# sebrahimi1988/dss-ml-at-scale

Hardware: AMD Instinct MI355X
Metric: samples/sec (higher is better)
Workload: dtype bf16; 1 GPU; model=resnet18, global_batch=212, parallelism=dp1+hipgraph

## Files before the change

mi355x_scale/models/resnet.py:

```python
from __future__ import annotations

from typing import List, Optional, Type, Union

import torch
import torch.nn as nn

from ..ops.conv3x3 import Conv3x3
from ..ops.fused_bn import FusedBNReLU2d
from ..ops.maxpool import MaxPool3x3s2
from ..ops.stemconv import StemConv2d


def _conv3x3(cin: int, cout: int, stride: int = 1) -> nn.Conv2d:
    if stride == 1 and cin == cout:
        return Conv3x3(cin, cout)
    return nn.Conv2d(cin, cout, 3, stride=stride, padding=1, bias=False)


def _conv1x1(cin: int, cout: int, stride: int = 1) -> nn.Conv2d:
    return nn.Conv2d(cin, cout, 1, stride=stride, bias=False)


class BasicBlock(nn.Module):
    expansion = 1
# ... 48 lines not shown
        self.layer3 = self._make_layer(block, 256, layers[2], stride=2)
        self.layer4 = self._make_layer(block, 512, layers[3], stride=2)
        self.avgpool = nn.AdaptiveAvgPool2d(1)
        self.fc = nn.Linear(512 * block.expansion, num_classes)

        for m in self.modules():
            if isinstance(m, nn.Conv2d):
                nn.init.kaiming_normal_(m.weight, mode="fan_out",
                                        nonlinearity="relu")
            elif isinstance(m, nn.BatchNorm2d):
                nn.init.ones_(m.weight)
                nn.init.zeros_(m.bias)
        if zero_init_residual:
            for m in self.modules():
                if isinstance(m, Bottleneck):
                    nn.init.zeros_(m.bn3.weight)
                elif isinstance(m, BasicBlock):
                    nn.init.zeros_(m.bn2.weight)

    def _make_layer(self, block, planes: int, blocks: int,
                    stride: int = 1) -> nn.Sequential:
        downsample = None
        if stride != 1 or self.inplanes != planes * block.expansion:
            downsample = nn.Sequential(
                _conv1x1(self.inplanes, planes * block.expansion, stride),
                FusedBNReLU2d(planes * block.expansion, relu=False),
            )
        layers = [block(self.inplanes, planes, stride, downsample)]
        self.inplanes = planes * block.expansion
        layers += [block(self.inplanes, planes) for _ in range(1, blocks)]
        return nn.Sequential(*layers)

    def forward(self, x: torch.Tensor) -> torch.Tensor:
        x = self.bn1.forward_pooled(self.conv1(x))
        x = self.layer4(self.layer3(self.layer2(self.layer1(x))))
        x = self.avgpool(x).flatten(1)
        return self.fc(x)


def resnet18(num_classes: int = 1000) -> ResNet:
    return ResNet(BasicBlock, [2, 2, 2, 2], num_classes)


def resnet34(num_classes: int = 1000) -> ResNet:
    return ResNet(BasicBlock, [3, 4, 6, 3], num_classes)


def resnet50(num_classes: int = 1000) -> ResNet:
    return ResNet(Bottleneck, [3, 4, 6, 3], num_classes)


MODELS = {"resnet18": resnet18, "resnet34": resnet34, "resnet50": resnet50}


def build_model(name: str, num_classes: int = 1000) -> ResNet:
    try:
        return MODELS[name](num_classes)
    except KeyError:
        raise ValueError(f"unknown model {name!r}; have {sorted(MODELS)}")
```

mi355x_scale/ops/csrc/bindings.cpp:

```cpp

#include <torch/extension.h>
#include <ATen/hip/HIPContext.h>
#include <hip/hip_runtime.h>

extern "C" void launch_normalize_u8_to_bf16(
    const uint8_t* in, void* out, const float* scale_dev,
    const float* shift_dev, long long n, hipStream_t stream);

void normalize_u8_to_bf16(torch::Tensor in, torch::Tensor out,
                          torch::Tensor scale, torch::Tensor shift) {
  TORCH_CHECK(in.is_cuda() && out.is_cuda(), "tensors must be on GPU");
  TORCH_CHECK(in.scalar_type() == torch::kUInt8, "input must be uint8");
  TORCH_CHECK(out.scalar_type() == torch::kBFloat16, "output must be bf16");
  TORCH_CHECK(in.is_contiguous(), "input must be contiguous (NHWC)");
  TORCH_CHECK(in.numel() == out.numel(), "element count mismatch");
  TORCH_CHECK(scale.is_cuda() && shift.is_cuda() && scale.numel() == 3 &&
                  shift.numel() == 3,
              "scale/shift must be 3-element device float tensors");
  TORCH_CHECK(scale.scalar_type() == torch::kFloat32 &&
              shift.scalar_type() == torch::kFloat32,
              "scale/shift must be float32");
  auto stream = at::cuda::getCurrentHIPStream();
  launch_normalize_u8_to_bf16(
      in.data_ptr<uint8_t>(), out.data_ptr(),
      scale.data_ptr<float>(), shift.data_ptr<float>(),
      (long long)in.numel(), stream.stream());
}

extern "C" void launch_groupfit_eval(
    const float* yT, const float* xc0, const float* xc1, const float* xc2,
    const float* pj0, const float* pj1, const float* pj2, const int* orders,
    float* mse, unsigned char* statusv,
    const float* b0, const float* b1, const float* b2,
    const float* w0, const float* w1, const float* w2,
    int T, long long G, int S, int C,
    int KX, hipStream_t stream);

extern "C" void launch_diff_center(const float* yT, float* wc, float* wm,
                                   int T, long long G, int S, int d,
                                   hipStream_t stream);

extern "C" void launch_exog_project_mfma(const float* P, const float* wc,
                                         float* beta, int n, long long G,
                                         int KX, hipStream_t stream);

extern "C" void launch_groupfit_final(
    const float* yT, const float* xc0, const float* xc1, const float* xc2,
    const float* pj0, const float* pj1, const float* pj2,
    const int* best_order, float* fitted, float* params,
    unsigned char* statusv,
    const float* b0, const float* b1, const float* b2,
    const float* w0, const float* w1, const float* w2,
    int T, long long G, int KX, hipStream_t stream);

extern "C" void launch_stem_conv_fwd(const void* x, const void* w, void* out,
                                     void* wp_scratch,
                                     int Nb, int H, int W, int HO, int WO,
                                     hipStream_t stream, int phase_mask);
extern "C" void launch_stem_conv_wrw(const void* x, const void* dy,
                                     float* dw_f32, void* dw_bf16,
                                     int Nb, int H, int W, int HO, int WO,
                                     hipStream_t stream, int phase_mask);
extern "C" void launch_conv3x3_wrw(const void* x, const void* dy,
                                   float* part, void* dw_bf16,
                                   int Nb, int H, int W, int C,
                                   int chunks, hipStream_t stream,
                                   int phase_mask);
extern "C" int conv3x3_wrw_chunks(int Nb, int H, int C, int chunks_req);

static void _check_f32(const torch::Tensor& t, const char* name) {
  TORCH_CHECK(t.is_cuda() && t.scalar_type() == torch::kFloat32 &&
                  t.is_contiguous(),
              name, " must be contiguous f32 on GPU");
}

void groupfit_eval(torch::Tensor yT, torch::Tensor xc0, torch::Tensor xc1,
                   torch::Tensor xc2, torch::Tensor pj0, torch::Tensor pj1,
                   torch::Tensor pj2, torch::Tensor orders,
                   torch::Tensor mse, torch::Tensor status, int64_t S,
                   torch::Tensor b0, torch::Tensor b1, torch::Tensor b2,
                   torch::Tensor w0, torch::Tensor w1, torch::Tensor w2) {
  _check_f32(yT, "yT"); _check_f32(xc0, "xc0"); _check_f32(xc1, "xc1");
  _check_f32(xc2, "xc2"); _check_f32(pj0, "pj0"); _check_f32(pj1, "pj1");
  _check_f32(pj2, "pj2"); _check_f32(mse, "mse");
  TORCH_CHECK(orders.scalar_type() == torch::kInt32 && orders.is_cuda());
  TORCH_CHECK(status.scalar_type() == torch::kUInt8 && status.is_cuda());
  int T = yT.size(0);
  long long G = yT.size(1);
  int C = orders.size(0);
  TORCH_CHECK(S > 8 && S <= T, "need 8 < S <= T");
  TORCH_CHECK(mse.size(0) == C && mse.size(1) == G);
// ... 490 lines not shown
                   at::cuda::getCurrentHIPStream().stream());
}

extern "C" void launch_adam_step_mixed(float* master, const void* gb,
                                       const float* gf, float* m, float* v,
                                       void* pb, int* step, float lr,
                                       float beta1, float beta2, float eps,
                                       float weight_decay, long long nb,
                                       long long n, hipStream_t stream);

void adam_step_mixed(torch::Tensor master, torch::Tensor gb,
                     torch::Tensor gf, torch::Tensor m, torch::Tensor v,
                     torch::Tensor pb, torch::Tensor step, double lr,
                     double beta1, double beta2, double eps,
                     double weight_decay) {
  _check_f32(master, "master"); _check_f32(m, "m"); _check_f32(v, "v");
  TORCH_CHECK(gb.scalar_type() == torch::kBFloat16 &&
              pb.scalar_type() == torch::kBFloat16, "gb/pb must be bf16");
  TORCH_CHECK(step.is_cuda() && step.scalar_type() == torch::kInt32 &&
              step.numel() == 1, "step must be int32[1] on device");
  long long n = master.numel();
  long long nb = gb.numel();
  TORCH_CHECK(pb.numel() == nb && gf.numel() == n - nb &&
              m.numel() == n && v.numel() == n, "buffer length mismatch");
  const float* gf_p = gf.numel() ? gf.data_ptr<float>() : nullptr;
  launch_adam_step_mixed(master.data_ptr<float>(), gb.data_ptr(), gf_p,
                         m.data_ptr<float>(), v.data_ptr<float>(),
                         pb.data_ptr(), step.data_ptr<int>(), (float)lr,
                         (float)beta1, (float)beta2, (float)eps,
                         (float)weight_decay, nb, n,
                         at::cuda::getCurrentHIPStream().stream());
}

void stem_conv_fwd(torch::Tensor x, torch::Tensor w, torch::Tensor out,
                   torch::Tensor wp_scratch, int64_t phase_mask = 7) {
  TORCH_CHECK(x.is_cuda() && x.scalar_type() == torch::kBFloat16);
  TORCH_CHECK(w.is_cuda() && w.scalar_type() == torch::kBFloat16);
  TORCH_CHECK(out.is_cuda() && out.scalar_type() == torch::kBFloat16);
  int Nb = x.size(0), H = x.size(1), W = x.size(2);
  TORCH_CHECK(x.size(3) == 3 && out.size(3) == 64, "stem is 3->64");
  int HO = out.size(1), WO = out.size(2);
  TORCH_CHECK(WO <= 128, "stem kernel handles output rows up to 128 px");
  TORCH_CHECK(w.numel() == 64 * 7 * 7 * 3);
  TORCH_CHECK(wp_scratch.scalar_type() == torch::kBFloat16 &&
              wp_scratch.numel() == 64 * 160);
  launch_stem_conv_fwd(x.data_ptr(), w.data_ptr(), out.data_ptr(),
                       wp_scratch.data_ptr(),
                       Nb, H, W, HO, WO,
                       at::cuda::getCurrentHIPStream().stream(),
                       (int)phase_mask);
}

void stem_conv_wrw(torch::Tensor x, torch::Tensor dy, torch::Tensor dw_f32,
                   torch::Tensor dw, int64_t phase_mask = 7) {
  TORCH_CHECK(x.is_cuda() && x.scalar_type() == torch::kBFloat16);
  TORCH_CHECK(dy.is_cuda() && dy.scalar_type() == torch::kBFloat16);
  TORCH_CHECK(dw_f32.scalar_type() == torch::kFloat32 &&
              dw_f32.numel() == 64 * 160);
  TORCH_CHECK(dw.scalar_type() == torch::kBFloat16 &&
              dw.numel() == 64 * 7 * 7 * 3);
  int Nb = x.size(0), H = x.size(1), W = x.size(2);
  int HO = dy.size(1), WO = dy.size(2);
  launch_stem_conv_wrw(x.data_ptr(), dy.data_ptr(),
                       dw_f32.data_ptr<float>(), dw.data_ptr(),
                       Nb, H, W, HO, WO,
                       at::cuda::getCurrentHIPStream().stream(),
                       (int)phase_mask);
}

void conv3x3_wrw(torch::Tensor x, torch::Tensor dy, torch::Tensor part,
                 torch::Tensor dw, int64_t phase_mask = 7,
                 int64_t chunks = 0) {
  TORCH_CHECK(x.is_cuda() && x.scalar_type() == torch::kBFloat16);
  TORCH_CHECK(dy.is_cuda() && dy.scalar_type() == torch::kBFloat16);
  int Nb = x.size(0), H = x.size(1), W = x.size(2), C = x.size(3);
  TORCH_CHECK(dy.size(1) == H && dy.size(2) == W && dy.size(3) == C,
              "same-shape 3x3 s1 conv only");
  TORCH_CHECK(C % 64 == 0 && C <= 2048, "C must be a multiple of 64");
  TORCH_CHECK(W >= 3 && W <= 64, "row length outside kernel bounds");
  const int nch = conv3x3_wrw_chunks(Nb, H, C, (int)chunks);
  TORCH_CHECK(part.scalar_type() == torch::kFloat32 &&
              part.numel() >= (long long)nch * C * 9 * C,
              "partial buffer too small for ", nch, " chunks");
  TORCH_CHECK(dw.scalar_type() == torch::kBFloat16 &&
              dw.numel() == (long long)C * 9 * C);
  launch_conv3x3_wrw(x.data_ptr(), dy.data_ptr(), part.data_ptr<float>(),
                     dw.data_ptr(), Nb, H, W, C, nch,
                     at::cuda::getCurrentHIPStream().stream(),
                     (int)phase_mask);
}

int64_t conv3x3_wrw_nchunks(int64_t Nb, int64_t H, int64_t C,
                            int64_t chunks) {
  return conv3x3_wrw_chunks((int)Nb, (int)H, (int)C, (int)chunks);
}

PYBIND11_MODULE(TORCH_EXTENSION_NAME, m) {
  m.def("conv3x3_wrw", &conv3x3_wrw,
        "MFMA 3x3/s1 CxC weight grad (fp32 accum, bf16 cast to view)",
        pybind11::arg("x"), pybind11::arg("dy"), pybind11::arg("part"),
        pybind11::arg("dw"), pybind11::arg("phase_mask") = 7,
        pybind11::arg("chunks") = 0);
  m.def("conv3x3_wrw_nchunks", &conv3x3_wrw_nchunks,
        "partial-buffer chunk count the wrw launcher will use");
  m.def("stem_conv_fwd", &stem_conv_fwd,
        "MFMA stem conv fwd (7x7 s2, 3->64, NHWC bf16)",
        pybind11::arg("x"), pybind11::arg("w"), pybind11::arg("out"),
        pybind11::arg("wp_scratch"), pybind11::arg("phase_mask") = 7);
  m.def("stem_conv_wrw", &stem_conv_wrw,
        "MFMA stem conv weight-grad (fp32 accum + bf16 cast)",
        pybind11::arg("x"), pybind11::arg("dy"), pybind11::arg("dw_f32"),
        pybind11::arg("dw"), pybind11::arg("phase_mask") = 7);
  m.def("normalize_u8_to_bf16", &normalize_u8_to_bf16,
        "fused uint8 NHWC -> normalized bf16 (same memory order)");
  m.def("groupfit_eval", &groupfit_eval,
        "batched per-group ARIMAX candidate evaluation (validation MSE)");
  m.def("groupfit_final", &groupfit_final,
        "batched per-group final fit (fitted values + params)");
  m.def("diff_center", &diff_center,
        "difference + per-group centering of the time-major panel");
  m.def("exog_project_mfma", &exog_project_mfma,
        "design-matrix GEMM beta = P @ Wc on f32 MFMA");
  m.def("bn_fwd_reduce", &bn_fwd_reduce);
  m.def("bn_fwd_finalize", &bn_fwd_finalize,
        "mean/invstd + running stats (+ optional int64 step counter)",
        pybind11::arg("partial"), pybind11::arg("mean"),
        pybind11::arg("invstd"), pybind11::arg("running_mean"),
        pybind11::arg("running_var"), pybind11::arg("momentum"),
        pybind11::arg("eps"), pybind11::arg("rows"), pybind11::arg("C"),
        pybind11::arg("update_running"),
        pybind11::arg("num_batches_tracked") = pybind11::none());
  m.def("bn_fwd_apply", &bn_fwd_apply);
  m.def("bn_bwd_reduce", &bn_bwd_reduce);
  m.def("bn_bwd_reduce_rm", &bn_bwd_reduce_rm);
  m.def("bn_bwd_apply_rm", &bn_bwd_apply_rm);
  m.def("bn_bwd_finalize", &bn_bwd_finalize);
  m.def("bn_bwd_apply", &bn_bwd_apply);
  m.def("bn_bwd_apply_dym", &bn_bwd_apply_dym);
  m.def("adam_step", &adam_step,
        "fused flat Adam step (one kernel over p/g/m/v)");
  m.def("maxpool3x3s2_fwd", &maxpool3x3s2_fwd);
// ... 12 lines not shown
```

mi355x_scale/ops/csrc/fused_bn.hip:

```cpp

#include <hip/hip_runtime.h>
#include <hip/hip_bf16.h>

typedef __hip_bfloat16 bf16;

#define VEC 8

union BVec {
  uint4 u;
  bf16 h[VEC];
};

static __device__ __forceinline__ BVec load8(const bf16* p) {
  BVec v;
  v.u = *reinterpret_cast<const uint4*>(p);
  return v;
}

static __device__ __forceinline__ void store8(bf16* p, const BVec& v) {
  *reinterpret_cast<uint4*>(p) = v.u;
}

__global__ __launch_bounds__(256) void bn_fwd_reduce_kernel(
    const bf16* __restrict__ x, float* __restrict__ partial,
// ... 10 lines not shown
    BVec v = load8(x + row * C + (long long)lane * VEC);
#pragma unroll
    for (int j = 0; j < VEC; ++j) {
      float f = __bfloat162float(v.h[j]);
      s[j] += f;
      q[j] += f * f;
    }
  }

  __shared__ float lds[256 * 2 * VEC];
  float* mys = &lds[(rsub * lanes + lane) * 2 * VEC];
#pragma unroll
  for (int j = 0; j < VEC; ++j) {
    mys[j] = s[j];
    mys[VEC + j] = q[j];
  }
  __syncthreads();
  for (int step = rows_per_iter >> 1; step > 0; step >>= 1) {
    if (rsub < step) {
      const float* other = &lds[((rsub + step) * lanes + lane) * 2 * VEC];
#pragma unroll
      for (int j = 0; j < 2 * VEC; ++j) mys[j] += other[j];
    }
    __syncthreads();
  }
  if (rsub == 0) {
#pragma unroll
    for (int j = 0; j < VEC; ++j) {
      partial[(long long)(lane * VEC + j) * gridDim.x + blockIdx.x] = mys[j];
      partial[(long long)(C + lane * VEC + j) * gridDim.x + blockIdx.x] =
          mys[VEC + j];
    }
  }
}

__global__ __launch_bounds__(256) void bn_fwd_finalize_kernel(
    const float* __restrict__ partial, int nblocks,
    float* __restrict__ mean, float* __restrict__ invstd,
    float* __restrict__ running_mean, float* __restrict__ running_var,
    float momentum, float eps, long long rows, int C, int update_running,
    long long* __restrict__ num_batches_tracked) {
  int c = blockIdx.x * (blockDim.x / 64) + threadIdx.x / 64;
  int lane = threadIdx.x % 64;
  if (c >= C) return;
  float s = 0.f, q = 0.f;
  for (int b = lane; b < nblocks; b += 64) {
    s += partial[(long long)c * nblocks + b];
    q += partial[(long long)(C + c) * nblocks + b];
  }
#pragma unroll
  for (int off = 32; off > 0; off >>= 1) {
    s += __shfl_down(s, off, 64);
    q += __shfl_down(q, off, 64);
  }
  if (lane != 0) return;
  float n = (float)rows;
  float m = s / n;
  float var = fmaxf(q / n - m * m, 0.f);
  mean[c] = m;
  invstd[c] = rsqrtf(var + eps);
  if (update_running) {
    float unbiased = rows > 1 ? var * (n / (n - 1.f)) : var;
    running_mean[c] = (1.f - momentum) * running_mean[c] + momentum * m;
    running_var[c] = (1.f - momentum) * running_var[c] + momentum * unbiased;
  }
  if (c == 0 && num_batches_tracked) *num_batches_tracked += 1;
}

template <bool RELU, bool RES>
__global__ __launch_bounds__(256) void bn_fwd_apply_kernel(
    const bf16* __restrict__ x, const bf16* __restrict__ res,
    bf16* __restrict__ y, const float* __restrict__ mean,
    const float* __restrict__ invstd, const float* __restrict__ weight,
    const float* __restrict__ bias, long long rows, int C) {
  const int lanes = C / VEC;
  const int lane = threadIdx.x % lanes;
  const int rsub = threadIdx.x / lanes;
  const int rows_per_iter = blockDim.x / lanes;
  const long long rstride = (long long)gridDim.x * rows_per_iter;

  float a[VEC], b[VEC];
#pragma unroll
  for (int j = 0; j < VEC; ++j) {
    int c = lane * VEC + j;
    a[j] = weight[c] * invstd[c];
    b[j] = bias[c] - mean[c] * a[j];
  }

  for (long long row = (long long)blockIdx.x * rows_per_iter + rsub;
       row < rows; row += rstride) {
    const long long off = row * C + (long long)lane * VEC;
    BVec v = load8(x + off);
    BVec r;
    if (RES) r = load8(res + off);
    BVec o;
#pragma unroll
    for (int j = 0; j < VEC; ++j) {
      float f = fmaf(__bfloat162float(v.h[j]), a[j], b[j]);
      if (RES) f += __bfloat162float(r.h[j]);
// ... 485 lines not shown
      for (int j = 0; j < VEC; ++j) {
        float xhat = (__bfloat162float(xv[p].h[j]) - m[j]) * is[j];
        float dy = rm_masked_dy(t.a[p][j], wv[j], xhat, bv[j]);
        float v = rm_dx(wis[j], dy, k1[j], xhat, k2[j]);
        odx.h[j] = __float2bfloat16(v);
      }
      store8(dx + t.pix[p], odx);
    }
  }
}


static int pick_grid(long long rows, int C) {
  int rows_per_iter = 256 / (C / VEC);
  long long blocks = (rows + rows_per_iter - 1) / rows_per_iter;
  if (blocks > 2080) blocks = 2080;
  return (int)(blocks > 0 ? blocks : 1);
}

extern "C" int bn_reduce_blocks(long long rows, int C) {
  int rows_per_iter = 256 / (C / VEC);
  long long blocks = (rows + rows_per_iter - 1) / rows_per_iter;
  if (blocks > 512) blocks = 512;
  return (int)(blocks > 0 ? blocks : 1);
}

extern "C" void launch_bn_fwd_reduce(const void* x, float* partial,
                                     int nblocks, long long rows, int C,
                                     hipStream_t stream) {
  hipLaunchKernelGGL(bn_fwd_reduce_kernel, dim3(nblocks), dim3(256), 0,
                     stream, (const bf16*)x, partial, rows, C);
}

extern "C" void launch_bn_fwd_finalize(const float* partial, int nblocks,
                                       float* mean, float* invstd,
                                       float* running_mean,
                                       float* running_var, float momentum,
                                       float eps, long long rows, int C,
                                       int update_running,
                                       long long* num_batches_tracked,
                                       hipStream_t stream) {
  hipLaunchKernelGGL(bn_fwd_finalize_kernel, dim3((C + 3) / 4),
                     dim3(256), 0, stream, partial, nblocks, mean, invstd,
                     running_mean, running_var, momentum, eps, rows, C,
                     update_running, num_batches_tracked);
}

extern "C" void launch_bn_fwd_apply(const void* x, const void* res, void* y,
                                    const float* mean, const float* invstd,
                                    const float* weight, const float* bias,
                                    long long rows, int C, int relu,
                                    hipStream_t stream) {
  dim3 grid(pick_grid(rows, C)), block(256);
#define APPLY(R, S)                                                       \
  hipLaunchKernelGGL((bn_fwd_apply_kernel<R, S>), grid, block, 0, stream, \
                     (const bf16*)x, (const bf16*)res, (bf16*)y, mean,    \
                     invstd, weight, bias, rows, C)
  if (relu && res) APPLY(true, true);
  else if (relu) APPLY(true, false);
  else if (res) APPLY(false, true);
  else APPLY(false, false);
#undef APPLY
}

extern "C" void launch_bn_bwd_reduce(const void* dz, const void* y,
                                     const void* x, const float* mean,
                                     const float* invstd, float* partial,
                                     void* dym, int nblocks, long long rows,
                                     int C, int relu, hipStream_t stream) {
  dim3 grid(nblocks), block(256);
#define REDUCE(R, W)                                                       \
  hipLaunchKernelGGL((bn_bwd_reduce_kernel<R, W>), grid, block, 0, stream, \
                     (const bf16*)dz, (const bf16*)y, (const bf16*)x,      \
                     mean, invstd, partial, (bf16*)dym, rows, C)
// ... 97 lines not shown
```

mi355x_scale/ops/csrc/stemconv.hip:

```cpp
#include <hip/hip_runtime.h>
#include <hip/hip_bf16.h>

#define KH 7
#define KW 7
#define CI 3
#define CO 64
#define KTAP (KH * KW * CI)
#define KPAD 160
#define KLDS 168
#define PXPAD 128
#define XTROW ((4 + 2 * PXPAD + KW + 4) * CI + 3)
#define XTOFF 12
#define STRIDE 2
#define PADDING 3

typedef __bf16 bf16;
typedef __attribute__((ext_vector_type(8))) __bf16 bf16x8;
typedef __attribute__((ext_vector_type(4))) __bf16 bf16x4;
typedef __attribute__((ext_vector_type(4))) float f32x4;

__device__ __forceinline__ void stage_band(
    const bf16* __restrict__ x, bf16* xt, int n, int ho, int H, int W,
    int tid, int nthreads, bool prime) {
  const int rowlen = W * CI;
// ... 142 lines not shown
    bf16x8 bfrag[4];
#pragma unroll
    for (int c = 0; c < 4; ++c)
      bfrag[c] = *reinterpret_cast<const bf16x8*>(
          wp + (c * 16 + row16) * KPAD + kk * 32 + kgrp * 8);
    bf16x8 f0, f1;
#pragma unroll
    for (int j = 0; j < 8; ++j) {
      const int ko = koff_of(kk * 32 + kgrp * 8 + j);
      f0[j] = xt[ko + pxb0];
      f1[j] = xt[ko + pxb1];
    }
#pragma unroll
    for (int c = 0; c < 4; ++c) {
      acc[0][c] = __builtin_amdgcn_mfma_f32_16x16x32_bf16(
          f0, bfrag[c], acc[0][c], 0, 0, 0);
      acc[1][c] = __builtin_amdgcn_mfma_f32_16x16x32_bf16(
          f1, bfrag[c], acc[1][c], 0, 0, 0);
    }
  }

  const long long rowbase = ((long long)n * HO + ho) * WO;
#pragma unroll
  for (int m = 0; m < 2; ++m) {
    const int pxr = wave * 32 + m * 16 + kgrp * 4;
#pragma unroll
    for (int r = 0; r < 4; ++r) {
      const int px = pxr + r;
      if (px >= WO) continue;
#pragma unroll
      for (int c = 0; c < 4; ++c)
        out[(rowbase + px) * CO + c * 16 + row16] = (bf16)acc[m][c][r];
    }
  }
}

extern "C" __global__ __launch_bounds__(256) void stem_conv_wrw_kernel(
    const bf16* __restrict__ x,
    const bf16* __restrict__ dy,
    float* __restrict__ dw,
    int Nb, int H, int W, int HO, int WO, int rows_per_block,
    int phase_mask) {
  __shared__ bf16 xt[8 * XTROW];
  __shared__ bf16 Dy[2 * PXPAD * CO];
  const int tid = threadIdx.x;
  const int wave = tid >> 6;
  const int lane = tid & 63;
  const int row16 = lane & 15;
  const int kgrp = lane >> 4;
  const int nrows = Nb * HO;
  const int mw = (wave >> 1) * 2;
  const int cw = (wave & 1) * 5;
  const int row_limit = min((blockIdx.x + 1) * rows_per_block, nrows);
  const int nch = (WO * CO) >> 3;
  const bf16x8 zv = {(bf16)0.0f, (bf16)0.0f, (bf16)0.0f, (bf16)0.0f,
                     (bf16)0.0f, (bf16)0.0f, (bf16)0.0f, (bf16)0.0f};

  f32x4 acc[2][5];
#pragma unroll
  for (int m = 0; m < 2; ++m)
#pragma unroll
    for (int c = 0; c < 5; ++c) acc[m][c] = (f32x4)0.0f;

  int cur = 0;
  {
    const int row0 = blockIdx.x * rows_per_block;
// ... 78 lines not shown
          acc[m][c] = __builtin_amdgcn_mfma_f32_16x16x32_bf16(
              afrag[m], bfr, acc[m][c], 0, 0, 0);
      }
    }
    if (have_next) {
      bf16x8* d8 = reinterpret_cast<bf16x8*>(Dy + (cur ^ 1) * PXPAD * CO);
#pragma unroll
      for (int u = 0; u < 4; ++u) d8[tid + u * 256] = v[u];
      cur ^= 1;
    }
  }

#pragma unroll
  for (int m = 0; m < 2; ++m)
#pragma unroll
    for (int c = 0; c < 5; ++c)
#pragma unroll
      for (int r = 0; r < 4; ++r) {
        const int co = (mw + m) * 16 + kgrp * 4 + r;
        const int k = (cw + c) * 16 + row16;
        atomicAdd(&dw[co * KPAD + k], acc[m][c][r]);
      }
}

extern "C" __global__ __launch_bounds__(256) void stem_wrw_cast_kernel(
    const float* __restrict__ dw, bf16* __restrict__ out) {
  const int i = blockIdx.x * 256 + threadIdx.x;
  if (i < CO * KTAP) {
    const int co = i / KTAP, k = i - co * KTAP;
    out[i] = (bf16)dw[co * KPAD + k];
  }
}

extern "C" void launch_stem_conv_fwd(const void* x, const void* w, void* out,
                                     void* wp_scratch,
                                     int Nb, int H, int W, int HO, int WO,
                                     hipStream_t stream, int phase_mask) {
  hipLaunchKernelGGL(stem_pad_weights_kernel,
                     dim3((CO * KPAD + 255) / 256), dim3(256), 0, stream,
                     (const bf16*)w, (bf16*)wp_scratch);
  hipLaunchKernelGGL(stem_conv_fwd_kernel, dim3(Nb * HO), dim3(256), 0,
                     stream, (const bf16*)x, (const bf16*)wp_scratch,
                     (bf16*)out, Nb, H, W, HO, WO, phase_mask);
}

extern "C" void launch_stem_conv_wrw(const void* x, const void* dy,
                                     float* dw_f32, void* dw_bf16,
                                     int Nb, int H, int W, int HO, int WO,
                                     hipStream_t stream,
                                     int phase_mask = 7) {
  const int nrows = Nb * HO;
  const int target_blocks = 768;
  const int rpb = (nrows + target_blocks - 1) / target_blocks;
  const int blocks = (nrows + rpb - 1) / rpb;
  hipMemsetAsync(dw_f32, 0, CO * KPAD * sizeof(float), stream);
  hipLaunchKernelGGL(stem_conv_wrw_kernel, dim3(blocks), dim3(256), 0,
                     stream, (const bf16*)x, (const bf16*)dy, dw_f32,
                     Nb, H, W, HO, WO, rpb, phase_mask);
  hipLaunchKernelGGL(stem_wrw_cast_kernel,
                     dim3((CO * KTAP + 255) / 256), dim3(256), 0, stream,
                     dw_f32, (bf16*)dw_bf16);
}
```

mi355x_scale/ops/fused_bn.py:

```python
from __future__ import annotations

from typing import Optional

import torch
import torch.nn as nn
import torch.nn.functional as F

from . import _C, require_ext


def _hip_supported(x: torch.Tensor) -> bool:
    c = x.shape[1]
    return (x.is_cuda and x.dtype == torch.bfloat16 and x.dim() == 4
            and c % 8 == 0 and c <= 2048 and (256 % (c // 8)) == 0)


class _FusedBNFn(torch.autograd.Function):
    @staticmethod
    def forward(ctx, x, residual, weight, bias, running_mean, running_var,
                momentum, eps, relu, num_batches_tracked):
        C = x.shape[1]
        rows = x.numel() // C
        dev = x.device
        mean = torch.empty(C, dtype=torch.float32, device=dev)
# ... 39 lines not shown
        dx = torch.empty_like(x)
        if ctx.has_res:
            dym = torch.empty_like(x)
            partial = _C.bn_bwd_reduce(dz, y, x, mean, invstd, dym, C,
                                       ctx.relu)
            _C.bn_bwd_finalize(partial, invstd, weight, dweight, dbias, k,
                               rows, C, fuse_acc)
            _C.bn_bwd_apply_dym(dym, x, mean, invstd, k, dx, C)
            return (dx, dym, None if fuse_acc else dweight,
                    None if fuse_acc else dbias, None, None, None, None,
                    None, None)
        if ctx.relu:
            partial = _C.bn_bwd_reduce_rm(dz, x, mean, invstd, weight,
                                          bias, x.new_empty(0), C)
            _C.bn_bwd_finalize(partial, invstd, weight, dweight, dbias, k,
                               rows, C, fuse_acc)
            _C.bn_bwd_apply_rm(dz, x, mean, invstd, bias, k, dx, C)
        else:
            partial = _C.bn_bwd_reduce(dz, y, x, mean, invstd,
                                       x.new_empty(0), C, False)
            _C.bn_bwd_finalize(partial, invstd, weight, dweight, dbias, k,
                               rows, C, fuse_acc)
            _C.bn_bwd_apply(dz, y, x, mean, invstd, k, dx, x.new_empty(0),
                            C, False)
        return (dx, None, None if fuse_acc else dweight,
                None if fuse_acc else dbias, None, None, None, None, None,
                None)


class _FusedBNPoolFn(torch.autograd.Function):

    @staticmethod
    def forward(ctx, x, weight, bias, running_mean, running_var,
                momentum, eps, training, num_batches_tracked):
        C = x.shape[1]
        dev = x.device
        if training:
            rows = x.numel() // C
            mean = torch.empty(C, dtype=torch.float32, device=dev)
            invstd = torch.empty(C, dtype=torch.float32, device=dev)
            partial = _C.bn_fwd_reduce(x, C)
            _C.bn_fwd_finalize(partial, mean, invstd, running_mean,
                               running_var, momentum, eps, rows, C, True,
                               num_batches_tracked)
        else:
            mean = running_mean.to(torch.float32)
            invstd = torch.rsqrt(running_var.to(torch.float32) + eps)
        n, _, h, w = x.shape
        ho, wo = (h + 1) // 2, (w + 1) // 2
        y = torch.empty((n, C, ho, wo), dtype=x.dtype, device=dev,
                        memory_format=torch.channels_last)
        code = torch.empty(n * ho * wo * C, dtype=torch.uint8, device=dev)
        _C.bn_maxpool3x3s2_fwd(x, mean, invstd, weight, bias, y, code)
        ctx.save_for_backward(x, mean, invstd, weight, bias, code)
        return y

    @staticmethod
    def backward(ctx, dp):
        x, mean, invstd, weight, bias, code = ctx.saved_tensors
        C = x.shape[1]
        rows = x.numel() // C
        dev = x.device
        if not dp.is_contiguous(memory_format=torch.channels_last):
            dp = dp.contiguous(memory_format=torch.channels_last)
        import os
        fused_unpool = os.environ.get("MI355X_BN_POOL_FUSED_BWD", "1") != "0"
        k = torch.empty(3 * C, dtype=torch.float32, device=dev)

        def _grad_view(p):
            g = p.grad
            if (g is not None and g.is_cuda and g.is_contiguous()
                    and g.dtype == torch.float32 and g.numel() == C):
                return g
            return None

        wg, bg = _grad_view(weight), _grad_view(bias)
        fuse_acc = (torch.cuda.is_current_stream_capturing()
                    and wg is not None and bg is not None
                    and os.environ.get("MI355X_BN_FUSED_ACC", "1") == "1")
        if fuse_acc:
            dweight, dbias = wg, bg
        else:
            dweight = torch.empty(C, dtype=torch.float32, device=dev)
            dbias = torch.empty(C, dtype=torch.float32, device=dev)
        dx = torch.empty_like(x)
        if fused_unpool:
            partial = _C.bn_pool_bwd_reduce(dp, code, x, mean, invstd,
                                            weight, bias)
            _C.bn_bwd_finalize(partial, invstd, weight, dweight, dbias, k,
                               rows, C, fuse_acc)
            _C.bn_pool_bwd_apply(dp, code, x, mean, invstd, bias, k, dx)
        else:
            dz = torch.empty_like(x)
            _C.maxpool3x3s2_bwd(dp, code, dz)
            partial = _C.bn_bwd_reduce_rm(dz, x, mean, invstd, weight, bias,
                                          x.new_empty(0), C)
            _C.bn_bwd_finalize(partial, invstd, weight, dweight, dbias, k,
                               rows, C, fuse_acc)
            _C.bn_bwd_apply_rm(dz, x, mean, invstd, bias, k, dx, C)
        return (dx, None if fuse_acc else dweight,
                None if fuse_acc else dbias, None, None, None, None, None,
                None)


class FusedBNReLU2d(nn.Module):

    gpu_fallbacks: list = []

    def __init__(self, num_features: int, eps: float = 1e-5,
                 momentum: float = 0.1, relu: bool = True):
        super().__init__()
        self.num_features = num_features
        self.eps = eps
        self.momentum = momentum
        self.relu = relu
        self.weight = nn.Parameter(torch.ones(num_features))
        self.bias = nn.Parameter(torch.zeros(num_features))
        self.register_buffer("running_mean", torch.zeros(num_features))
        self.register_buffer("running_var", torch.ones(num_features))
        self.register_buffer("num_batches_tracked",
                             torch.tensor(0, dtype=torch.long))

    def extra_repr(self) -> str:
        return (f"{self.num_features}, eps={self.eps}, "
                f"momentum={self.momentum}, relu={self.relu}")

    def forward_pooled(self, x: torch.Tensor) -> torch.Tensor:
        assert self.relu, "pooled fusion is relu-only"
        if _hip_supported(x):
            require_ext()
            x = x.contiguous(memory_format=torch.channels_last)
            return _FusedBNPoolFn.apply(
                x, self.weight, self.bias, self.running_mean,
                self.running_var, self.momentum, self.eps, self.training,
                self.num_batches_tracked)
        return F.max_pool2d(self.forward(x), 3, stride=2, padding=1)

    def forward(self, x: torch.Tensor,
                residual: Optional[torch.Tensor] = None) -> torch.Tensor:
        if _hip_supported(x):
            require_ext()
            x = x.contiguous(memory_format=torch.channels_last)
            if residual is not None:
                residual = residual.contiguous(
                    memory_format=torch.channels_last)
            if self.training:
                return _FusedBNFn.apply(
                    x, residual, self.weight, self.bias, self.running_mean,
                    self.running_var, self.momentum, self.eps, self.relu,
                    self.num_batches_tracked)
            if not (torch.is_grad_enabled() and
                    (x.requires_grad or self.weight.requires_grad)):
                invstd = torch.rsqrt(self.running_var + self.eps)
                y = torch.empty_like(x)
                res = (residual if residual is not None else x.new_empty(0))
                _C.bn_fwd_apply(x, res, y, self.running_mean, invstd,
                                self.weight, self.bias, x.shape[1],
                                self.relu)
                return y
        if self.training:
            self.num_batches_tracked += 1
        if x.is_cuda and len(FusedBNReLU2d.gpu_fallbacks) < 256:
            FusedBNReLU2d.gpu_fallbacks.append(
                (tuple(x.shape), str(x.dtype), self.training))
        y = F.batch_norm(x, self.running_mean, self.running_var, self.weight,
                         self.bias, self.training, self.momentum, self.eps)
        if residual is not None:
            y = y + residual
# ... 2 lines not shown
```

mi355x_scale/ops/stemconv.py:

```python
from __future__ import annotations

import os

import torch
import torch.nn as nn
import torch.nn.functional as F


class _StemConvFn(torch.autograd.Function):
    @staticmethod
    def forward(ctx, x: torch.Tensor, weight: torch.Tensor):
        from . import _C
        N, C, H, W = x.shape
        HO = (H + 2 * 3 - 7) // 2 + 1
        WO = (W + 2 * 3 - 7) // 2 + 1
        out = torch.empty((N, 64, HO, WO), dtype=torch.bfloat16,
                          device=x.device,
                          memory_format=torch.channels_last)
        wp = torch.empty(64 * 160, dtype=torch.bfloat16, device=x.device)
        _C.stem_conv_fwd(x.permute(0, 2, 3, 1), weight.permute(0, 2, 3, 1),
                         out.permute(0, 2, 3, 1), wp)
        ctx.save_for_backward(x, weight)
        return out

    @staticmethod
    def backward(ctx, dy: torch.Tensor):
        from . import _C
        x, weight = ctx.saved_tensors
        if dy.dtype != torch.bfloat16:
            dy = dy.to(torch.bfloat16)
        dy = dy.contiguous(memory_format=torch.channels_last)
        dw = torch.empty_like(weight)
        scratch = torch.empty(64 * 160, dtype=torch.float32,
                              device=x.device)
        _C.stem_conv_wrw(x.permute(0, 2, 3, 1), dy.permute(0, 2, 3, 1),
                         scratch, dw.permute(0, 2, 3, 1))
        return None, dw


class StemConv2d(nn.Conv2d):

    def __init__(self):
        super().__init__(3, 64, 7, stride=2, padding=3, bias=False)

    def _hip_ok(self, x: torch.Tensor) -> bool:
        from . import HAVE_EXT
        return (HAVE_EXT and x.is_cuda
                and os.environ.get("MI355X_STEM_CONV", "1") == "1"
                and x.shape[-1] <= 262
                and x.dtype == torch.bfloat16
                and self.weight.dtype == torch.bfloat16
                and x.is_contiguous(memory_format=torch.channels_last)
                and self.weight.is_contiguous(
                    memory_format=torch.channels_last)
                and not x.requires_grad)

    def forward(self, x: torch.Tensor) -> torch.Tensor:
        if self._hip_ok(x):
            return _StemConvFn.apply(x, self.weight)
        if x.is_cuda and torch.cuda.is_available():
            from . import HAVE_EXT, require_ext
            if HAVE_EXT is False and x.dtype == torch.bfloat16:
                require_ext()
        return F.conv2d(x, self.weight, None, self.stride, self.padding)
```

Measured before the change: 26310 samples/s.

## Fuse BN statistics reduction into stem conv forward kernel

Result: faster. 26880 samples/s, median of 6 (+2.1%).

```diff
diff --git a/mi355x_scale/models/resnet.py b/mi355x_scale/models/resnet.py
--- a/mi355x_scale/models/resnet.py
+++ b/mi355x_scale/models/resnet.py
@@ -104,7 +104,11 @@
         return nn.Sequential(*layers)
 
     def forward(self, x: torch.Tensor) -> torch.Tensor:
-        x = self.bn1.forward_pooled(self.conv1(x))
+        if self.bn1.training and self.conv1.stats_ok(x):
+            x, partial = self.conv1.forward_with_stats(x)
+            x = self.bn1.forward_pooled(x, partial)
+        else:
+            x = self.bn1.forward_pooled(self.conv1(x))
         x = self.layer4(self.layer3(self.layer2(self.layer1(x))))
         x = self.avgpool(x).flatten(1)
         return self.fc(x)
diff --git a/mi355x_scale/ops/csrc/bindings.cpp b/mi355x_scale/ops/csrc/bindings.cpp
--- a/mi355x_scale/ops/csrc/bindings.cpp
+++ b/mi355x_scale/ops/csrc/bindings.cpp
@@ -54,9 +54,10 @@
     int T, long long G, int KX, hipStream_t stream);
 
 extern "C" void launch_stem_conv_fwd(const void* x, const void* w, void* out,
-                                     void* wp_scratch,
+                                     void* wp_scratch, float* partial,
                                      int Nb, int H, int W, int HO, int WO,
                                      hipStream_t stream, int phase_mask);
+extern "C" int stem_fwd_stat_blocks(int Nb, int HO);
 extern "C" void launch_stem_conv_wrw(const void* x, const void* dy,
                                      float* dw_f32, void* dw_bf16,
                                      int Nb, int H, int W, int HO, int WO,
@@ -613,8 +614,13 @@
                          at::cuda::getCurrentHIPStream().stream());
 }
 
+int64_t stem_fwd_blocks(int64_t Nb, int64_t HO) {
+  return stem_fwd_stat_blocks((int)Nb, (int)HO);
+}
+
 void stem_conv_fwd(torch::Tensor x, torch::Tensor w, torch::Tensor out,
-                   torch::Tensor wp_scratch, int64_t phase_mask = 7) {
+                   torch::Tensor wp_scratch, int64_t phase_mask = 7,
+                   c10::optional<torch::Tensor> partial = c10::nullopt) {
   TORCH_CHECK(x.is_cuda() && x.scalar_type() == torch::kBFloat16);
   TORCH_CHECK(w.is_cuda() && w.scalar_type() == torch::kBFloat16);
   TORCH_CHECK(out.is_cuda() && out.scalar_type() == torch::kBFloat16);
@@ -625,8 +631,21 @@
   TORCH_CHECK(w.numel() == 64 * 7 * 7 * 3);
   TORCH_CHECK(wp_scratch.scalar_type() == torch::kBFloat16 &&
               wp_scratch.numel() == 64 * 160);
+  TORCH_CHECK(x.is_contiguous() && out.is_contiguous() &&
+                  out.size(0) == Nb && HO == (H - 1) / 2 + 1 &&
+                  WO == (W - 1) / 2 + 1,
+              "stem conv: dense NHWC x/out with 7x7 s2 p3 geometry");
+  float* partial_p = nullptr;
+  if (partial.has_value()) {
+    const torch::Tensor& p = *partial;
+    TORCH_CHECK(p.is_cuda() && p.scalar_type() == torch::kFloat32 &&
+                    p.is_contiguous() &&
+                    p.numel() == 2 * 64 * stem_fwd_blocks(Nb, HO),
+                "partial must be fp32 [2*64*stem_fwd_blocks(N, HO)]");
+    partial_p = p.data_ptr<float>();
+  }
   launch_stem_conv_fwd(x.data_ptr(), w.data_ptr(), out.data_ptr(),
-                       wp_scratch.data_ptr(),
+                       wp_scratch.data_ptr(), partial_p,
                        Nb, H, W, HO, WO,
                        at::cuda::getCurrentHIPStream().stream(),
                        (int)phase_mask);
@@ -687,7 +706,10 @@
   m.def("stem_conv_fwd", &stem_conv_fwd,
         "MFMA stem conv fwd (7x7 s2, 3->64, NHWC bf16)",
         pybind11::arg("x"), pybind11::arg("w"), pybind11::arg("out"),
-        pybind11::arg("wp_scratch"), pybind11::arg("phase_mask") = 7);
+        pybind11::arg("wp_scratch"), pybind11::arg("phase_mask") = 7,
+        pybind11::arg("partial") = pybind11::none());
+  m.def("stem_fwd_blocks", &stem_fwd_blocks,
+        "block (= BN partial slot) count of the fused-statistics stem fwd");
   m.def("stem_conv_wrw", &stem_conv_wrw,
         "MFMA stem conv weight-grad (fp32 accum + bf16 cast)",
         pybind11::arg("x"), pybind11::arg("dy"), pybind11::arg("dw_f32"),
diff --git a/mi355x_scale/ops/csrc/fused_bn.hip b/mi355x_scale/ops/csrc/fused_bn.hip
--- a/mi355x_scale/ops/csrc/fused_bn.hip
+++ b/mi355x_scale/ops/csrc/fused_bn.hip
@@ -66,6 +66,25 @@
           mys[VEC + j];
     }
   }
+}
+
+static __device__ __forceinline__ void bn_fwd_finalize_channel(
+    int c, float s, float q, float* __restrict__ mean,
+    float* __restrict__ invstd, float* __restrict__ running_mean,
+    float* __restrict__ running_var, float momentum, float eps,
+    long long rows, int update_running,
+    long long* __restrict__ num_batches_tracked) {
+  float n = (float)rows;
+  float m = s / n;
+  float var = fmaxf(q / n - m * m, 0.f);
+  mean[c] = m;
+  invstd[c] = rsqrtf(var + eps);
+  if (update_running) {
+    float unbiased = rows > 1 ? var * (n / (n - 1.f)) : var;
+    running_mean[c] = (1.f - momentum) * running_mean[c] + momentum * m;
+    running_var[c] = (1.f - momentum) * running_var[c] + momentum * unbiased;
+  }
+  if (c == 0 && num_batches_tracked) *num_batches_tracked += 1;
 }
 
 __global__ __launch_bounds__(256) void bn_fwd_finalize_kernel(
@@ -88,17 +107,53 @@
     q += __shfl_down(q, off, 64);
   }
   if (lane != 0) return;
-  float n = (float)rows;
-  float m = s / n;
-  float var = fmaxf(q / n - m * m, 0.f);
-  mean[c] = m;
-  invstd[c] = rsqrtf(var + eps);
-  if (update_running) {
-    float unbiased = rows > 1 ? var * (n / (n - 1.f)) : var;
-    running_mean[c] = (1.f - momentum) * running_mean[c] + momentum * m;
-    running_var[c] = (1.f - momentum) * running_var[c] + momentum * unbiased;
-  }
-  if (c == 0 && num_batches_tracked) *num_batches_tracked += 1;
+  bn_fwd_finalize_channel(c, s, q, mean, invstd, running_mean, running_var,
+                          momentum, eps, rows, update_running,
+                          num_batches_tracked);
+}
+
+__global__ __launch_bounds__(256) void bn_fwd_finalize_wide_kernel(
+    const float* __restrict__ partial, int nblocks,
+    float* __restrict__ mean, float* __restrict__ invstd,
+    float* __restrict__ running_mean, float* __restrict__ running_var,
+    float momentum, float eps, long long rows, int C, int update_running,
+    long long* __restrict__ num_batches_tracked) {
+  const int c = blockIdx.x;
+  const int tid = threadIdx.x;
+  const float* ps = partial + (long long)c * nblocks;
+  const float* pq = partial + (long long)(C + c) * nblocks;
+  float s4[4] = {0.f, 0.f, 0.f, 0.f}, q4[4] = {0.f, 0.f, 0.f, 0.f};
+  int b = tid;
+  for (; b + 3 * 256 < nblocks; b += 4 * 256) {
+#pragma unroll
+    for (int u = 0; u < 4; ++u) {
+      s4[u] += ps[b + u * 256];
+      q4[u] += pq[b + u * 256];
+    }
+  }
+  for (; b < nblocks; b += 256) {
+    s4[0] += ps[b];
+    q4[0] += pq[b];
+  }
+  float s = (s4[0] + s4[1]) + (s4[2] + s4[3]);
+  float q = (q4[0] + q4[1]) + (q4[2] + q4[3]);
+#pragma unroll
+  for (int off = 32; off > 0; off >>= 1) {
+    s += __shfl_down(s, off, 64);
+    q += __shfl_down(q, off, 64);
+  }
+  __shared__ float ws[4], wq[4];
+  if ((tid & 63) == 0) {
+    ws[tid >> 6] = s;
+    wq[tid >> 6] = q;
+  }
+  __syncthreads();
+  if (tid != 0) return;
+  s = (ws[0] + ws[1]) + (ws[2] + ws[3]);
+  q = (wq[0] + wq[1]) + (wq[2] + wq[3]);
+  bn_fwd_finalize_channel(c, s, q, mean, invstd, running_mean, running_var,
+                          momentum, eps, rows, update_running,
+                          num_batches_tracked);
 }
 
 template <bool RELU, bool RES>
@@ -650,6 +705,8 @@
                      stream, (const bf16*)x, partial, rows, C);
 }
 
+#define BN_FINALIZE_WIDE_MIN 1024
+
 extern "C" void launch_bn_fwd_finalize(const float* partial, int nblocks,
                                        float* mean, float* invstd,
                                        float* running_mean,
@@ -658,6 +715,13 @@
                                        int update_running,
                                        long long* num_batches_tracked,
                                        hipStream_t stream) {
+  if (nblocks > BN_FINALIZE_WIDE_MIN) {
+    hipLaunchKernelGGL(bn_fwd_finalize_wide_kernel, dim3(C), dim3(256), 0,
+                       stream, partial, nblocks, mean, invstd, running_mean,
+                       running_var, momentum, eps, rows, C, update_running,
+                       num_batches_tracked);
+    return;
+  }
   hipLaunchKernelGGL(bn_fwd_finalize_kernel, dim3((C + 3) / 4),
                      dim3(256), 0, stream, partial, nblocks, mean, invstd,
                      running_mean, running_var, momentum, eps, rows, C,
diff --git a/mi355x_scale/ops/csrc/stemconv.hip b/mi355x_scale/ops/csrc/stemconv.hip
--- a/mi355x_scale/ops/csrc/stemconv.hip
+++ b/mi355x_scale/ops/csrc/stemconv.hip
@@ -198,6 +198,182 @@
       for (int c = 0; c < 4; ++c)
         out[(rowbase + px) * CO + c * 16 + row16] = (bf16)acc[m][c][r];
     }
+  }
+}
+
+#define FWD_ROWS 8
+#define FWD_BAND_ROWS (2 * FWD_ROWS + KH - STRIDE)
+#define OTROW 72
+#define XTCH (XTROW / 4)
+#define STAGE_DEPTH 17
+
+__device__ __forceinline__ void stage_band_rows(
+    const bf16* __restrict__ x, bf16* xt, int n, int ih0, int nrows_in,
+    int H, int W, int tid, int nthreads) {
+  const int rowlen = W * CI;
+  if ((rowlen & 3) == 0) {
+    const int nch = rowlen >> 2;
+    const int total = nrows_in * XTCH;
+    const bf16x4 z = {(bf16)0.0f, (bf16)0.0f, (bf16)0.0f, (bf16)0.0f};
+    for (int base = 0; base < total; base += nthreads * STAGE_DEPTH) {
+      bf16x4 v[STAGE_DEPTH];
+#pragma unroll
+      for (int u = 0; u < STAGE_DEPTH; ++u) {
+        const int i = base + tid + u * nthreads;
+        v[u] = z;
+        if (i < total) {
+          const int r = i / XTCH, c = i - r * XTCH - XTOFF / 4;
+          const int ih = ih0 + r;
+          if (ih >= 0 && ih < H && c >= 0 && c < nch)
+            v[u] = reinterpret_cast<const bf16x4*>(
+                x + ((long long)n * H + ih) * rowlen)[c];
+        }
+      }
+#pragma unroll
+      for (int u = 0; u < STAGE_DEPTH; ++u) {
+        const int i = base + tid + u * nthreads;
+        if (i < total) reinterpret_cast<bf16x4*>(xt)[i] = v[u];
+      }
+    }
+  } else {
+    const int total = nrows_in * XTROW;
+    for (int i = tid; i < total; i += nthreads) {
+      const int r = i / XTROW, e = i - r * XTROW - XTOFF;
+      const int ih = ih0 + r;
+      bf16 v = (bf16)0.0f;
+      if (ih >= 0 && ih < H && e >= 0 && e < rowlen)
+        v = x[((long long)n * H + ih) * rowlen + e];
+      xt[i] = v;
+    }
+  }
+}
+
+extern "C" __global__ __launch_bounds__(256, 3) void stem_conv_fwd_stats_kernel(
+    const bf16* __restrict__ x,
+    const bf16* __restrict__ wp,
+    bf16* __restrict__ out,
+    float* __restrict__ partial,
+    int Nb, int H, int W, int HO, int WO, int nchunks, int phase_mask) {
+  __shared__ __attribute__((aligned(16))) bf16 xt[FWD_BAND_ROWS * XTROW];
+  __shared__ __attribute__((aligned(16))) bf16 ot[4 * 32 * OTROW];
+  __shared__ __attribute__((aligned(16))) unsigned short ktab[4 * KPAD / 4];
+  const int tid = threadIdx.x;
+  const int wave = tid >> 6;
+  const int lane = tid & 63;
+  const int row16 = lane & 15;
+  const int kgrp = lane >> 4;
+  const int n = blockIdx.x / nchunks;
+  const int ho0 = (blockIdx.x - n * nchunks) * FWD_ROWS;
+  const int rows = min(FWD_ROWS, HO - ho0);
+
+  bf16x8 bfrag[KPAD / 32][4];
+#pragma unroll
+  for (int kk = 0; kk < KPAD / 32; ++kk)
+#pragma unroll
+    for (int c = 0; c < 4; ++c)
+      bfrag[kk][c] = *reinterpret_cast<const bf16x8*>(
+          wp + (c * 16 + row16) * KPAD + kk * 32 + kgrp * 8);
+
+  if (tid < 4 * KPAD / 4) {
+    const int g = tid / (KPAD / 4), i = tid - g * (KPAD / 4);
+    const int k = (i >> 3) * 32 + g * 8 + (i & 7);
+    ktab[tid] = (unsigned short)(2 * koff_of(min(k, KTAP - 1)));
+  }
+  if (phase_mask & 1)
+    stage_band_rows(x, xt, n, ho0 * STRIDE - PADDING,
+                    rows * STRIDE + KH - STRIDE, H, W, tid, 256);
+  __syncthreads();
+  if (!(phase_mask & 4)) return;
+
+  float ssum[4] = {0.f, 0.f, 0.f, 0.f}, ssq[4] = {0.f, 0.f, 0.f, 0.f};
+  const int pxb0 = (wave * 32 + row16) * (STRIDE * CI);
+  const int pxb1 = (wave * 32 + 16 + row16) * (STRIDE * CI);
+  bf16* tw = ot + wave * 32 * OTROW;
+#pragma unroll 1
+  for (int rr = 0; rr < rows; ++rr) {
+    const int rshift = rr * STRIDE * XTROW;
+#pragma unroll 1
+    for (int m = 0; m < 2; ++m) {
+      f32x4 acc[4];
+#pragma unroll
+      for (int c = 0; c < 4; ++c) acc[c] = (f32x4)0.0f;
+      const unsigned rb = 2u * (unsigned)(rshift + (m ? pxb1 : pxb0));
+      const uint4* tp = reinterpret_cast<const uint4*>(ktab) + kgrp * 5;
+      asm volatile("" : "+v"(tp));
+#pragma unroll
+      for (int kk = 0; kk < KPAD / 32; ++kk) {
+        const uint4 t4 = tp[kk];
+        const unsigned tk[4] = {t4.x, t4.y, t4.z, t4.w};
+        bf16x8 f;
+#pragma unroll
+        for (int j = 0; j < 8; ++j) {
+          const int k = kk * 32 + kgrp * 8 + j;
+          const bool kz = (kk == KPAD / 32 - 1) && k >= KTAP;
+          const unsigned pk = tk[j >> 1];
+          const unsigned ob = ((j & 1) ? (pk >> 16) : (pk & 0xffffu)) + rb;
+          f[j] = *reinterpret_cast<const bf16*>(
+              reinterpret_cast<const char*>(xt) + (kz ? 0u : ob));
+        }
+#pragma unroll
+        for (int c = 0; c < 4; ++c)
+          acc[c] = __builtin_amdgcn_mfma_f32_16x16x32_bf16(
+              f, bfrag[kk][c], acc[c], 0, 0, 0);
+      }
+#pragma unroll
+      for (int r = 0; r < 4; ++r) {
+        const int pxl = m * 16 + kgrp * 4 + r;
+        const bool live = wave * 32 + pxl < WO;
+#pragma unroll
+        for (int c = 0; c < 4; ++c) {
+          const bf16 v = (bf16)acc[c][r];
+          tw[pxl * OTROW + c * 16 + row16] = v;
+          const float f = live ? (float)v : 0.f;
+          ssum[c] += f;
+          ssq[c] += f * f;
+        }
+      }
+    }
+    __builtin_amdgcn_fence(__ATOMIC_RELEASE, "wavefront");
+    __builtin_amdgcn_wave_barrier();
+    __builtin_amdgcn_fence(__ATOMIC_ACQUIRE, "wavefront");
+    const long long rowbase = ((long long)n * HO + ho0 + rr) * WO;
+#pragma unroll
+    for (int t = 0; t < 4; ++t) {
+      const int v = lane + t * 64;
+      const int pxl = v >> 3, j8 = (v & 7) * 8;
+      const int px = wave * 32 + pxl;
+      const bf16x8 val = *reinterpret_cast<const bf16x8*>(
+          tw + pxl * OTROW + j8);
+      if (px < WO)
+        *reinterpret_cast<bf16x8*>(out + (rowbase + px) * CO + j8) = val;
+    }
+    __builtin_amdgcn_fence(__ATOMIC_RELEASE, "wavefront");
+    __builtin_amdgcn_wave_barrier();
+    __builtin_amdgcn_fence(__ATOMIC_ACQUIRE, "wavefront");
+  }
+
+#pragma unroll
+  for (int c = 0; c < 4; ++c) {
+    ssum[c] += __shfl_xor(ssum[c], 16, 64);
+    ssum[c] += __shfl_xor(ssum[c], 32, 64);
+    ssq[c] += __shfl_xor(ssq[c], 16, 64);
+    ssq[c] += __shfl_xor(ssq[c], 32, 64);
+  }
+  float* red = reinterpret_cast<float*>(tw);
+  if (kgrp == 0) {
+#pragma unroll
+    for (int c = 0; c < 4; ++c) {
+      red[c * 16 + row16] = ssum[c];
+      red[CO + c * 16 + row16] = ssq[c];
+    }
+  }
+  __syncthreads();
+  if (tid < 2 * CO) {
+    float t = 0.f;
+#pragma unroll
+    for (int w = 0; w < 4; ++w)
+      t += reinterpret_cast<const float*>(ot + w * 32 * OTROW)[tid];
+    partial[(long long)tid * gridDim.x + blockIdx.x] = t;
   }
 }
 
@@ -342,13 +518,25 @@
   }
 }
 
+extern "C" int stem_fwd_stat_blocks(int Nb, int HO) {
+  return Nb * ((HO + FWD_ROWS - 1) / FWD_ROWS);
+}
+
 extern "C" void launch_stem_conv_fwd(const void* x, const void* w, void* out,
-                                     void* wp_scratch,
+                                     void* wp_scratch, float* partial,
                                      int Nb, int H, int W, int HO, int WO,
                                      hipStream_t stream, int phase_mask) {
   hipLaunchKernelGGL(stem_pad_weights_kernel,
                      dim3((CO * KPAD + 255) / 256), dim3(256), 0, stream,
                      (const bf16*)w, (bf16*)wp_scratch);
+  if (partial) {
+    const int nchunks = (HO + FWD_ROWS - 1) / FWD_ROWS;
+    hipLaunchKernelGGL(stem_conv_fwd_stats_kernel, dim3(Nb * nchunks),
+                       dim3(256), 0, stream, (const bf16*)x,
+                       (const bf16*)wp_scratch, (bf16*)out, partial,
+                       Nb, H, W, HO, WO, nchunks, phase_mask);
+    return;
+  }
   hipLaunchKernelGGL(stem_conv_fwd_kernel, dim3(Nb * HO), dim3(256), 0,
                      stream, (const bf16*)x, (const bf16*)wp_scratch,
                      (bf16*)out, Nb, H, W, HO, WO, phase_mask);
diff --git a/mi355x_scale/ops/fused_bn.py b/mi355x_scale/ops/fused_bn.py
--- a/mi355x_scale/ops/fused_bn.py
+++ b/mi355x_scale/ops/fused_bn.py
@@ -95,14 +95,15 @@
 
     @staticmethod
     def forward(ctx, x, weight, bias, running_mean, running_var,
-                momentum, eps, training, num_batches_tracked):
+                momentum, eps, training, num_batches_tracked, partial=None):
         C = x.shape[1]
         dev = x.device
         if training:
             rows = x.numel() // C
             mean = torch.empty(C, dtype=torch.float32, device=dev)
             invstd = torch.empty(C, dtype=torch.float32, device=dev)
-            partial = _C.bn_fwd_reduce(x, C)
+            if partial is None:
+                partial = _C.bn_fwd_reduce(x, C)
             _C.bn_fwd_finalize(partial, mean, invstd, running_mean,
                                running_var, momentum, eps, rows, C, True,
                                num_batches_tracked)
@@ -163,7 +164,7 @@
             _C.bn_bwd_apply_rm(dz, x, mean, invstd, bias, k, dx, C)
         return (dx, None if fuse_acc else dweight,
                 None if fuse_acc else dbias, None, None, None, None, None,
-                None)
+                None, None)
 
 
 class FusedBNReLU2d(nn.Module):
@@ -188,7 +189,9 @@
         return (f"{self.num_features}, eps={self.eps}, "
                 f"momentum={self.momentum}, relu={self.relu}")
 
-    def forward_pooled(self, x: torch.Tensor) -> torch.Tensor:
+    def forward_pooled(self, x: torch.Tensor,
+                       partial: Optional[torch.Tensor] = None
+                       ) -> torch.Tensor:
         assert self.relu, "pooled fusion is relu-only"
         if _hip_supported(x):
             require_ext()
@@ -196,7 +199,8 @@
             return _FusedBNPoolFn.apply(
                 x, self.weight, self.bias, self.running_mean,
                 self.running_var, self.momentum, self.eps, self.training,
-                self.num_batches_tracked)
+                self.num_batches_tracked,
+                partial if self.training else None)
         return F.max_pool2d(self.forward(x), 3, stride=2, padding=1)
 
     def forward(self, x: torch.Tensor,
diff --git a/mi355x_scale/ops/stemconv.py b/mi355x_scale/ops/stemconv.py
--- a/mi355x_scale/ops/stemconv.py
+++ b/mi355x_scale/ops/stemconv.py
@@ -7,35 +7,69 @@
 import torch.nn.functional as F
 
 
+def fused_stats_enabled() -> bool:
+    return os.environ.get("MI355X_STEM_FUSED_STATS", "1") != "0"
+
+
+def _stem_forward(x: torch.Tensor, weight: torch.Tensor, fused: bool):
+    from . import _C
+    N, C, H, W = x.shape
+    HO = (H + 2 * 3 - 7) // 2 + 1
+    WO = (W + 2 * 3 - 7) // 2 + 1
+    out = torch.empty((N, 64, HO, WO), dtype=torch.bfloat16,
+                      device=x.device,
+                      memory_format=torch.channels_last)
+    wp = torch.empty(64 * 160, dtype=torch.bfloat16, device=x.device)
+    partial = None
+    if fused:
+        partial = torch.empty(2 * 64 * _C.stem_fwd_blocks(N, HO),
+                              dtype=torch.float32, device=x.device)
+    _C.stem_conv_fwd(x.permute(0, 2, 3, 1), weight.permute(0, 2, 3, 1),
+                     out.permute(0, 2, 3, 1), wp, 7, partial)
+    return out, partial
+
+
+def _stem_backward(ctx, dy: torch.Tensor):
+    from . import _C
+    x, weight = ctx.saved_tensors
+    if dy.dtype != torch.bfloat16:
+        dy = dy.to(torch.bfloat16)
+    dy = dy.contiguous(memory_format=torch.channels_last)
+    dw = torch.empty_like(weight)
+    scratch = torch.empty(64 * 160, dtype=torch.float32,
+                          device=x.device)
+    _C.stem_conv_wrw(x.permute(0, 2, 3, 1), dy.permute(0, 2, 3, 1),
+                     scratch, dw.permute(0, 2, 3, 1))
+    return None, dw
+
+
 class _StemConvFn(torch.autograd.Function):
     @staticmethod
     def forward(ctx, x: torch.Tensor, weight: torch.Tensor):
-        from . import _C
-        N, C, H, W = x.shape
-        HO = (H + 2 * 3 - 7) // 2 + 1
-        WO = (W + 2 * 3 - 7) // 2 + 1
-        out = torch.empty((N, 64, HO, WO), dtype=torch.bfloat16,
-                          device=x.device,
-                          memory_format=torch.channels_last)
-        wp = torch.empty(64 * 160, dtype=torch.bfloat16, device=x.device)
-        _C.stem_conv_fwd(x.permute(0, 2, 3, 1), weight.permute(0, 2, 3, 1),
-                         out.permute(0, 2, 3, 1), wp)
+        out, _ = _stem_forward(x, weight, fused_stats_enabled())
         ctx.save_for_backward(x, weight)
         return out
 
     @staticmethod
     def backward(ctx, dy: torch.Tensor):
-        from . import _C
-        x, weight = ctx.saved_tensors
-        if dy.dtype != torch.bfloat16:
-            dy = dy.to(torch.bfloat16)
-        dy = dy.contiguous(memory_format=torch.channels_last)
-        dw = torch.empty_like(weight)
-        scratch = torch.empty(64 * 160, dtype=torch.float32,
-                              device=x.device)
-        _C.stem_conv_wrw(x.permute(0, 2, 3, 1), dy.permute(0, 2, 3, 1),
-                         scratch, dw.permute(0, 2, 3, 1))
-        return None, dw
+        return _stem_backward(ctx, dy)
+
+
+class _StemConvStatsFn(torch.autograd.Function):
+
+    @staticmethod
+    def forward(ctx, x: torch.Tensor, weight: torch.Tensor):
+        out, partial = _stem_forward(x, weight, True)
+        ctx.save_for_backward(x, weight)
+        ctx.mark_non_differentiable(partial)
+        ctx.set_materialize_grads(False)
+        return out, partial
+
+    @staticmethod
+    def backward(ctx, dy, _dpartial):
+        if dy is None:
+            return None, None
+        return _stem_backward(ctx, dy)
 
 
 class StemConv2d(nn.Conv2d):
@@ -55,6 +89,14 @@
                     memory_format=torch.channels_last)
                 and not x.requires_grad)
 
+    def stats_ok(self, x: torch.Tensor) -> bool:
+        return fused_stats_enabled() and self._hip_ok(x)
+
+    def forward_with_stats(self, x: torch.Tensor):
+        if self.stats_ok(x):
+            return _StemConvStatsFn.apply(x, self.weight)
+        return self.forward(x), None
+
     def forward(self, x: torch.Tensor) -> torch.Tensor:
         if self._hip_ok(x):
             return _StemConvFn.apply(x, self.weight)
```
